# michaelosthege/pytensor-federated

Measured on NVIDIA H100. Metric: logp+grad evals/sec for 8-shard federated GLM, higher is better.
Workload: dtype bf16; 1 GPU; model=federated logistic GLM (logp + gradient), chains_per_eval=1, features=256, global_batch=80000000, seq_len=256, l2_policy=inputs (>= 2.5 GB per GPU) are larger than the 50 MB L2; no flush needed, parallelism=shard-parallel x1 (8 shards/GPU), kernel=auto, backend=fused, comm=local, hbm_bytes_per_eval_per_gpu=31200395264

## Files before the change

pytensor_federated_b200/csrc/glm_tc.cu:

```cuda
#include <cstring>
#include <vector>

#include <cuda.h>
#include <cuda_bf16.h>
#include <cuda_runtime.h>

#include "fed_comm.cuh"
#include "models.h"
#include "tc_common.cuh"
#include "chunks.h"

namespace tc {

constexpr int kTileM = 128;
constexpr int kPanel = 64;
constexpr int kPanelBytes = kTileM * 128;
constexpr int kThreads = 512;
constexpr int kRegs = 65536 / kThreads;
constexpr int kConsumerRegs = 168;
constexpr int kOtherRegs = 88;
static_assert(256 * kConsumerRegs + 256 * kOtherRegs == 65536, "the register split must fill the register file");
constexpr int kConsumerWarps = 8;
constexpr int kMaxChunk = 32;
constexpr int kMinChunk = 4;
constexpr int kRing = 16;
constexpr int kLLRows = 16;

constexpr int kXBlock = kTileM * kPanel * 3 / 2;
constexpr int kXFoot = 256;
constexpr int kXMaxExceptions = kXFoot / 4 - 1;
constexpr int kXSlots = 6;
constexpr int kDecThreads = 224;

__host__ __device__ __forceinline__ uint32_t x12_prmt(uint32_t a, uint32_t b, uint32_t s) {
#ifdef __CUDA_ARCH__
    uint32_t r;
    asm("prmt.b32 %0, %1, %2, %3;" : "=r"(r) : "r"(a), "r"(b), "r"(s));
    return r;
#else
    const uint64_t v = (uint64_t)b << 32 | a;
    uint32_t r = 0;
    for (int k = 0; k < 4; ++k) {
        const uint32_t sel = (s >> (4 * k)) & 0xFu;
        uint32_t byte = (uint32_t)(v >> (8 * (sel & 7u))) & 0xFFu;
        if (sel & 8u) byte = (byte & 0x80u) ? 0xFFu : 0u;
        r |= byte << (8 * k);
    }
    return r;
#endif
}
__host__ __device__ __forceinline__ uint4 x12_decode8(uint2 lo, uint32_t c, const uint32_t (&t)[4]) {
    const uint32_t w = c << 4;
    const uint32_t s0 = c & 0x7777u, s1 = (c >> 16) & 0x7777u;
    const uint32_t m0 = x12_prmt(w, c, 0xD9C8u), m1 = x12_prmt(w, c, 0xFBEAu);
    const uint32_t h0 = (x12_prmt(t[0], t[1], s0) & ~m0) | (x12_prmt(t[2], t[3], s0) & m0);
    const uint32_t h1 = (x12_prmt(t[0], t[1], s1) & ~m1) | (x12_prmt(t[2], t[3], s1) & m1);
    uint4 r;
    r.x = x12_prmt(lo.x, h0, 0x5140u);
    r.y = x12_prmt(lo.x, h0, 0x7362u);
    r.z = x12_prmt(lo.y, h1, 0x5140u);
    r.w = x12_prmt(lo.y, h1, 0x7362u);
    return r;
}
__host__ __device__ __forceinline__ uint32_t x12_chunk_offset(int i) { return (i >> 3) * 128 + (((i & 7) ^ ((i >> 3) & 7)) << 4); }
__host__ __device__ __forceinline__ uint32_t x12_high_byte_offset(uint32_t pos) {
    const uint32_t pnl = pos >> 13, row = (pos >> 6) & 127, f = pos & 63;
    return pnl * kPanelBytes + row * 128 + ((((f >> 3) ^ (row & 7)) << 4) | ((f & 7) << 1)) + 1;
}

struct SmemLayout {
    uint32_t stages, stage_bytes, off_theta_b, theta_b_bytes, off_r, r_bytes, off_rows, row_bytes, off_theta_f,
        off_disp, off_ring, off_bars, total, preload, xslots, xslot_bytes, off_x, off_xfoot;
};
__host__ __device__ inline SmemLayout smem_layout(int P, int n1, int n2, int n_theta, int chain_words, int chains,
                                                  int row_arrays, bool packed = false) {
    SmemLayout L;
    const uint32_t panels = P / kPanel;
    L.stage_bytes = panels * kPanelBytes;
    L.theta_b_bytes = panels * n1 * 128;
    L.r_bytes = kTileM * n2 * 2;
    L.row_bytes = (uint32_t)row_arrays * kTileM * 4;
    const uint32_t bars_bytes = packed ? 256 : 192;
    const uint32_t fixed = L.theta_b_bytes + 2 * L.r_bytes + ((chains * (1 + chain_words) * 4 + 15) & ~15) + kRing * 24 +
                           bars_bytes + (packed ? 2 * kXFoot : 0) + 1024 ;
    uint32_t stages = (227u * 1024u - fixed) / (L.stage_bytes + L.row_bytes);
    if (stages > 4) stages = 4;
    L.xslots = 0;
    L.xslot_bytes = kXBlock + kXFoot + L.row_bytes;
    if (packed) {
        const uint32_t two = fixed + 2 * (L.stage_bytes + L.row_bytes);
        stages = 2;
        if (two <= 227u * 1024u && (uint32_t)n_theta * 4u <= 2u * L.stage_bytes) {
            const uint32_t fit = (227u * 1024u - two) / L.xslot_bytes;
            L.xslots = fit < (uint32_t)kXSlots ? fit : (uint32_t)kXSlots;
        }
    }
    L.stages = stages;
// ... 126 lines not shown
    uint64_t* bar_xempty = bars + 20 + kXSlots;

    const int warp = threadIdx.x >> 5;
    const int lane = threadIdx.x & 31;

    if (threadIdx.x == 0) {
        *pipeline_fault() = 0;
        for (int i = 0; i < kRing; ++i) mbar_init(&bar_ring[i], 1);
        for (int i = 0; i < 4; ++i) { mbar_init(&bar_full[i], PK ? kDecThreads : 1); mbar_init(&bar_empty[i], 32 * kConsumerWarps); }
        if (PK)
            for (int i = 0; i < kXSlots; ++i) { mbar_init(&bar_xfull[i], 1); mbar_init(&bar_xempty[i], kDecThreads); }
        fence_barrier_init();
    }
    if (warp == 0 && lane == 0)
        for (int i = 0; i < prm.n_segments; ++i) {
            tma_prefetch_desc(&tmaps[4 * i]);
            tma_prefetch_desc(&tmaps[4 * i + 1]);
            if (ROWS && segs_g[i].offset) tma_prefetch_desc(&tmaps[4 * i + 2]);
            if (ROWS && segs_g[i].weight) tma_prefetch_desc(&tmaps[4 * i + 3]);
        }
    auto load_tile = [&](int st, int seg, int row0, int rows) {
        const CUtensorMap* m = tmaps + 4 * seg;
        float* slot = reinterpret_cast<float*>(smem + L.off_rows + (size_t)st * L.row_bytes);
        mbar_expect_tx(&bar_full[st], L.stage_bytes + kTileM * 4 * (1 + (rows & 1) + (rows >> 1)));
        for (int pnl = 0; pnl < panels; ++pnl)
            tma_load_2d(smem + (size_t)st * L.stage_bytes + pnl * kPanelBytes, m, pnl * kPanel, row0, &bar_full[st]);
        tma_load_1d(slot, m + 1, row0, &bar_full[st]);
        if (rows & 1) tma_load_1d(slot + o_slot * kTileM, m + 2, row0, &bar_full[st]);
        if (rows & 2) tma_load_1d(slot + w_slot * kTileM, m + 3, row0, &bar_full[st]);
    };
    auto load_xpanel = [&](int xs, int seg, int tile, int pnl, int rows) {
        unsigned char* dst = smem + L.off_x + (size_t)xs * L.xslot_bytes;
        const GlmSegment& g = segs_g[seg];
        const uint32_t extra = pnl == 0 ? kXFoot + kTileM * 4 * (1 + (rows & 1) + (rows >> 1)) : 0;
        mbar_expect_tx(&bar_xfull[xs], kXBlock + extra);
        bulk_load(dst, static_cast<const unsigned char*>(g.xpack) + ((size_t)tile * panels + pnl) * kXBlock, kXBlock, &bar_xfull[xs]);
        if (pnl == 0) {
            const CUtensorMap* m = tmaps + 4 * seg;
            float* slot = reinterpret_cast<float*>(dst + kXBlock + kXFoot);
            bulk_load(dst + kXBlock, static_cast<const unsigned char*>(g.xfoot) + (size_t)tile * kXFoot, kXFoot, &bar_xfull[xs]);
            tma_load_1d(slot, m + 1, tile * kTileM, &bar_xfull[xs]);
            if (rows & 1) tma_load_1d(slot + o_slot * kTileM, m + 2, tile * kTileM, &bar_xfull[xs]);
            if (rows & 2) tma_load_1d(slot + w_slot * kTileM, m + 3, tile * kTileM, &bar_xfull[xs]);
        }
    };
    auto seg_row_mask = [&](int seg) -> int {
        if constexpr (!ROWS) return 0;
        return (segs_g[seg].offset ? 1 : 0) | (segs_g[seg].weight ? 2 : 0);
    };
    unsigned int claim0 = 0;
    int preloaded = 0;
    if (warp == 0) {
        __syncwarp();
        fed::pdl_wait();
        if (lane == 0) claim0 = atomicAdd(work_counter, 1u);
        claim0 = __shfl_sync(0xffffffffu, claim0, 0);
        if (claim0 < (unsigned int)n_chunks) {
            const GlmChunk ch = chunks[claim0];
            const int units = PK ? ch.n_tiles * panels : ch.n_tiles;
            preloaded = units < (int)L.preload ? units : (int)L.preload;
            if (!prm.early_loads) preloaded = 0;
            const int rows = seg_row_mask(ch.seg);
            if (elect_one())
                for (int t = 0; t < preloaded; ++t) {
                    if (PK) load_xpanel(t, ch.seg, ch.first_tile + t / panels, t % panels, rows);
                    else load_tile(t, ch.seg, (ch.first_tile + t) * kTileM, rows);
                }
            __syncwarp();
        }
    }

    __shared__ fed::Prologue s_pro;
    bool active;
    {
// ... 83 lines not shown
                    }
                    __syncwarp();
                    if (!have) break;
                    const int rows = seg_row_mask(ch.seg);
                    for (int t = 0; t < ch.n_tiles && PK; ++t)
                        for (int pnl = 0; pnl < panels; ++pnl) {
                            const int k = t * panels + pnl;
                            if (!(j == 0 && k < preloaded)) {
                                mbar_wait(&bar_xempty[xs.idx], xs.phase ^ 1);
                                if (j == 0 && k == preloaded && lane == 0) fed::stamp(comm, 3);
                                if (elect_one()) load_xpanel(xs.idx, ch.seg, ch.first_tile + t, pnl, rows);
                                __syncwarp();
                            }
                            xs.advance((int)L.xslots);
                        }
                    for (int t = 0; t < ch.n_tiles && !PK; ++t) {
                        const int st = stage.idx;
                        if (j == 0 && t < preloaded) {
                            stage.advance(S);
                            continue;
                        }
                        mbar_wait(&bar_empty[st], stage.phase ^ 1);
                        if (j == 0 && t == preloaded && lane == 0) fed::stamp(comm, 3);
                        if (elect_one()) load_tile(st, ch.seg, (ch.first_tile + t) * kTileM, rows);
                        __syncwarp();
                        stage.advance(S);
                    }
                    claim = __shfl_sync(0xffffffffu, ahead, 0);
                }
                if (lane == 0) fed::stamp(comm, 4);
            } else {
                if (PK) {
                    const int td = warp < 4 ? threadIdx.x - 32 : threadIdx.x - (12 * 32 - 96);
                    constexpr int kDecGroup = KC <= 4 && traits(E).group_panels ? 2 : 1;
                    static_assert(kDecGroup <= 2, "a packed launch may have only 2 compressed slots");
                    int4* decided = reinterpret_cast<int4*>(smem + L.off_bars + 144);
                    Ring stage, xs;
                    uint32_t fb = 0;
                    for (int j = 0;; ++j) {
                        mbar_wait(&bar_ring[j & (kRing - 1)], (uint32_t)((j / kRing) & 1));
                        named_sync(2, kDecThreads);
                        if (td == 0) *decided = *pipeline_fault() ? make_int4(-1, 0, 0, 0) : ring[j & (kRing - 1)];
                        named_sync(2, kDecThreads);
                        const int4 ch = *decided;
                        if (ch.x < 0) break;
                        const uint32_t tab[4] = {segs_g[ch.x].xtab[0], segs_g[ch.x].xtab[1], segs_g[ch.x].xtab[2],
                                                 segs_g[ch.x].xtab[3]};
                        for (int t = 0; t < ch.z; ++t) {
                            mbar_wait(&bar_empty[stage.idx], stage.phase ^ 1);
                            unsigned char* dst = smem + (size_t)stage.idx * L.stage_bytes;
                            int* foot = reinterpret_cast<int*>(smem + L.off_xfoot + fb * kXFoot);
                            for (int pnl = 0; pnl < panels; pnl += kDecGroup) {
                                constexpr int kPer = (kTileM * 8 + kDecThreads - 1) / kDecThreads;
                                uint2 lo[kDecGroup][kPer];
                                uint32_t cw[kDecGroup][kPer];
                                int xi[kDecGroup];
#pragma unroll
                                for (int h = 0; h < kDecGroup; ++h) {
                                    mbar_wait(&bar_xfull[xs.idx], xs.phase);
                                    const unsigned char* src = smem + L.off_x + (size_t)xs.idx * L.xslot_bytes;
                                    if (pnl + h == 0) {
                                        if (td < kXFoot / 4) foot[td] = reinterpret_cast<const int*>(src + kXBlock)[td];
                                        const float* rsrc = reinterpret_cast<const float*>(src + kXBlock + kXFoot);
                                        float* rdst = reinterpret_cast<float*>(smem + L.off_rows + (size_t)stage.idx * L.row_bytes);
                                        for (int i = td; i < (int)L.row_bytes / 4; i += kDecThreads) rdst[i] = rsrc[i];
                                    }
#pragma unroll
                                    for (int k = 0; k < kPer; ++k) {
                                        const int i = td + k * kDecThreads;
                                        if (k < kPer - 1 || i < kTileM * 8) {
                                            lo[h][k] = reinterpret_cast<const uint2*>(src)[i];
                                            cw[h][k] = reinterpret_cast<const uint32_t*>(src + kTileM * kPanel)[i];
                                        }
                                    }
                                    xi[h] = xs.idx;
                                    xs.advance((int)L.xslots);
                                }
#pragma unroll
                                for (int h = 0; h < kDecGroup; ++h) {
                                    unsigned char* pd = dst + (pnl + h) * kPanelBytes;
#pragma unroll
                                    for (int k = 0; k < kPer; ++k) {
                                        const int i = td + k * kDecThreads;
                                        if (k < kPer - 1 || i < kTileM * 8)
                                            *reinterpret_cast<uint4*>(pd + x12_chunk_offset(i)) = x12_decode8(lo[h][k], cw[h][k], tab);
                                    }
                                    mbar_arrive(&bar_xempty[xi[h]]);
                                }
                            }
                            named_sync(2, kDecThreads);
                            const int n_ex = min(foot[0], kXMaxExceptions);
                            for (int e = td; e < n_ex; e += kDecThreads) {
                                const uint32_t v = (uint32_t)foot[1 + e];
                                if ((v >> 8) < (uint32_t)panels * kTileM * kPanel) dst[x12_high_byte_offset(v >> 8)] = (unsigned char)(v & 0xFFu);
                            }
                            fence_proxy_async();
                            mbar_arrive(&bar_full[stage.idx]);
                            stage.advance(S);
                            fb ^= 1u;
                        }
                    }
                }
            }
            named_sync(3, kThreads);
            setmaxnreg<kOtherRegs, kRegs>();
        } else {
            setmaxnreg<kRegs, kConsumerRegs>();
            const int c = (warp >> 2) - 1;
            const int w = warp & 3;
            const int q = lane & 3;
            const int ew = warp - 4;
            const int NB = PP / 128;
            constexpr int NJ = C8 / 8;
            const uint64_t desc_k = make_desc(0, 16, 1024, 1);
            const uint64_t desc_xt = make_desc(0, kPanelBytes, 1024, 1);
            const uint64_t desc_r = make_desc(0, 128, 2048, 0);
            const uint32_t theta_b_a = smem_u32(theta_b);
            const uint32_t x_base_a = smem_u32(smem);
            const uint32_t r_a = smem_u32(r_buf);
// ... 453 lines not shown
    return e == cudaSuccess ? 0 : (int)e;
}

extern "C" int b200_glm_tc_chunk_table(const long long* n_rows, int n_segments, int sm_count, int multiple, int max_chunk,
                                       int min_chunk, int* out, int max_chunks) {
    std::vector<GlmSegment> segs(n_segments);
    for (int s = 0; s < n_segments; ++s) segs[s].n_rows = n_rows[s];
    const std::vector<GlmChunk> chunks = build_chunks(segs.data(), n_segments, sm_count, tc::kTileM, multiple, max_chunk, min_chunk);
    for (size_t i = 0; i < chunks.size() && (int)i < max_chunks; ++i) {
        out[3 * i + 0] = chunks[i].seg;
        out[3 * i + 1] = chunks[i].first_tile;
        out[3 * i + 2] = chunks[i].n_tiles;
    }
    return (int)chunks.size();
}

extern "C" size_t b200_glm_tc_partial_row_doubles(int n_vals, int n_chains, int n_out, int n_groups, int family) {
    return tc::partial_row_doubles(n_vals, chains_bucket(n_chains), n_out > 0 ? n_out : 1, n_groups,
                                   tc::traits(tc::epilogue(family)).disp ? 1 : 0);
}

extern "C" int b200_glm_tc_stages(int n_features, int n_chains, int n_groups, int family, int row_data) {
    const int kc = chains_bucket(n_chains);
    if (kc == 0) return 0;
    return (int)launch_layout(n_features, kc, tc::epilogue(family), 0, row_data != 0, row_data).stages;
}

extern "C" int b200_glm_tc_packed_slots(int n_features, int n_chains, int n_groups, int family, int row_data, int n_theta) {
    const int kc = chains_bucket(n_chains);
    if (kc == 0) return 0;
    return (int)launch_layout(n_features, kc, tc::epilogue(family), n_theta, row_data != 0, row_data, true).xslots;
}

extern "C" int b200_glm_x12_decode_tile(const unsigned char* blocks, const int* footer, const unsigned int* tab, int panels,
                                        unsigned char* out) {
    const uint32_t t[4] = {tab[0], tab[1], tab[2], tab[3]};
    for (int pnl = 0; pnl < panels; ++pnl) {
        const unsigned char* src = blocks + (size_t)pnl * tc::kXBlock;
        for (int i = 0; i < tc::kTileM * 8; ++i) {
            uint2 lo;
            uint32_t c;
            std::memcpy(&lo, src + 8 * i, 8);
            std::memcpy(&c, src + tc::kTileM * tc::kPanel + 4 * i, 4);
            const uint4 v = tc::x12_decode8(lo, c, t);
            std::memcpy(out + (size_t)pnl * tc::kPanelBytes + tc::x12_chunk_offset(i), &v, 16);
        }
    }
    if (footer[0] < 0 || footer[0] > tc::kXMaxExceptions) return -1;
    for (int e = 0; e < footer[0]; ++e) {
        const uint32_t v = (uint32_t)footer[1 + e];
        if ((v >> 8) >= (uint32_t)panels * tc::kTileM * tc::kPanel) return -1;
        out[tc::x12_high_byte_offset(v >> 8)] = (unsigned char)(v & 0xFFu);
    }
    return footer[0];
}

extern "C" int b200_launch_glm_tc(const FedComm* comm, const GlmSegment* segs_dev, const GlmParams* prm, const void* tmaps,
                                  const void* chunks_dev, int n_chunks, unsigned int* work_counter, int grid,
                                  cudaStream_t stream) {
    const int kc = chains_bucket(prm->n_chains);
    if (kc == 0) return -1;
    const bool rows = prm->row_data != 0;
    const LaunchFn fn = pick(tc::epilogue(prm->family), kc, rows);
    if (!fn) return -3;
    return fn(comm, segs_dev, prm, tmaps, chunks_dev, n_chunks, work_counter, grid, stream);
}
```

pytensor_federated_b200/csrc/models.h:

```cpp
#pragma once
#include <cstdint>

struct LinregShard {
    const void* x;
    const void* y;
    long long n;
    double sigma;
    int theta_offset;
    int _pad;
};

struct GlmSegment {
    const void* X;
    const float* y;
    const void* scales;
    const float* offset;
    const float* weight;
    long long n_rows;
    long long first_tile;
    int group;
    int out_group;
    const void* xpack;
    const void* xfoot;
    unsigned int xtab[4];
};

struct GlmParams {
    int n_segments;
    int n_features;
    int ld;
    int n_groups;
    int n_chains;
    int family;
    long long total_tiles;
    int n_out;
    int early_loads;
    int row_data;
    int n_classes;
    int packed_x;
};

constexpr int kGlmRowOffsets = 1;
constexpr int kGlmRowWeights = 2;
constexpr int kGlmHvp = 16;

enum GlmFamilyCode : int {
    kGlmLogistic = 0,
    kGlmPoisson = 1,
    kGlmGaussian = 2,
    kGlmMultinomial = 3,
    kGlmGaussianScale = 4,
    kGlmNegBinomial = 5,
    kGlmOrdinal = 6,
    kGlmWeibull = 7,
    kGlmLogNormal = 8,
    kGlmZeroInflatedPoisson = 9,
    kGlmZeroInflatedNegBinomial = 10,
// ... 57 lines not shown
```

pytensor_federated_b200/csrc/runtime.cu:

```cuda
#include <atomic>
#include <chrono>
#include <cstdio>
#include <cstdlib>
#include <cstring>
#include <string>
#include <thread>
#include <vector>

#include <cuda_runtime.h>

#include "fed_comm.cuh"
#include "models.h"

static bool early_loads_enabled() {
    const char* v = getenv("B200FED_NO_EARLY_LOADS");
    return !(v && *v && *v != '0');
}

extern "C" {
int b200_launch_linreg(const FedComm*, const LinregShard*, int, int, int, cudaStream_t);
int b200_launch_glm_simt(const FedComm*, const GlmSegment*, const GlmParams*, int, cudaStream_t);
size_t b200_glm_simt_smem(int, int, int);
int b200_launch_glm_tc(const FedComm*, const GlmSegment*, const GlmParams*, const void* tmaps, const void* chunks,
                       int n_chunks, unsigned int* work_counter, int grid, cudaStream_t);
// ... 574 lines not shown
    CK(cudaMalloc((void**)&e->glm_segs_dev, sizeof(GlmSegment) * (n_segments > 0 ? n_segments : 1)));
    CK(cudaMemcpy(e->glm_segs_dev, e->glm_segs.data(), sizeof(GlmSegment) * n_segments, cudaMemcpyHostToDevice));
    if (use_tensor_cores == 3 || use_tensor_cores == 4) {
        e->glm_elem_bytes = use_tensor_cores == 3 ? 2 : 4;
        e->kind = MODEL_GLM_GENERIC;
        e->grid = e->sm_count * 2;
    } else if (use_tensor_cores) {
        const bool fp8 = use_tensor_cores == 2;
        if (fp8) {
            int rc = b200_glm_fp8_prepare(e->glm_segs.data(), n_segments, &e->glm, e->sm_count, &e->glm_tmaps_dev,
                                          &e->glm_chunks_dev, &e->glm_n_chunks);
            if (rc != 0) {
                g_last_error = "fp8 GLM path rejected this shape (rc=" + std::to_string(rc) + ")";
                return rc;
            }
        }
        e->tc_row_doubles = fp8 ? b200_glm_fp8_partial_row_doubles(e->n_vals, n_chains, e->glm.n_out, n_groups)
                                : b200_glm_tc_partial_row_doubles(e->n_vals, n_chains, e->glm.n_out, n_groups, family);
        if (e->tc_partials) cudaFree(e->tc_partials);
        const size_t doubles = (size_t)e->sm_count * e->tc_row_doubles + ((size_t)e->sm_count / 16 + 2) * e->n_vals * 2;
        CK(cudaMalloc((void**)&e->tc_partials, doubles * 8));
        CK(cudaMemset(e->tc_partials, 0, doubles * 8));
        e->kind = fp8 ? MODEL_GLM_FP8 : MODEL_GLM_TC;
        e->grid = e->sm_count;
        if (e->glm_n_chunks > 0 && e->grid > e->glm_n_chunks) e->grid = e->glm_n_chunks;
    } else {
        e->kind = MODEL_GLM_SIMT;
        e->grid = e->sm_count * 2;
    }
    if ((long long)e->grid > tiles && tiles > 0) e->grid = (int)tiles;
    return 0;
}

int b200_engine_set_glm_packed(void* h, int n_segments, const void** xpack, const void** xfoot, const unsigned int* tabs) {
    Engine* e = static_cast<Engine*>(h);
    CK(cudaSetDevice(e->device));
    if (e->kind != MODEL_GLM_TC || n_segments != (int)e->glm_segs.size()) {
        g_last_error = "packed X needs the bf16 tensor-core GLM model it was made for";
        return -41;
    }
    std::vector<GlmSegment> segs = e->glm_segs;
    for (int s = 0; s < n_segments; ++s) {
        segs[s].xpack = xpack ? xpack[s] : nullptr;
        segs[s].xfoot = xpack ? xfoot[s] : nullptr;
        for (int q = 0; q < 4; ++q) segs[s].xtab[q] = xpack ? tabs[4 * s + q] : 0u;
        if (xpack && (!segs[s].xpack || !segs[s].xfoot || (((uintptr_t)segs[s].xpack | (uintptr_t)segs[s].xfoot) & 15) != 0)) {
            g_last_error = "packed X: every segment needs 16-byte aligned blocks and footers";
            return -42;
        }
    }
    if (xpack && b200_glm_tc_packed_slots(e->glm.n_features, e->glm.n_chains, e->glm.n_groups, e->glm.family,
                                          e->glm.row_data, e->n_theta) < 2) {
        g_last_error = "packed X: this shape's packed layout does not fit in shared memory";
        return -43;
    }
    CK(cudaMemcpy(e->glm_segs_dev, segs.data(), sizeof(GlmSegment) * n_segments, cudaMemcpyHostToDevice));
    e->glm_segs = segs;
    e->glm.packed_x = xpack ? 1 : 0;
    return 0;
}

void b200_engine_set_custom_launcher(void* h, void* fn) {
    static_cast<Engine*>(h)->custom_launcher =
        reinterpret_cast<int (*)(const FedComm*, const GlmSegment*, const GlmParams*, int, int, cudaStream_t)>(fn);
}

void b200_engine_set_ode_launcher(void* h, void* fn) {
    static_cast<Engine*>(h)->ode_launcher =
        reinterpret_cast<int (*)(const FedComm*, const OdeShard*, int, int, cudaStream_t)>(fn);
}

int b200_engine_set_ode(void* h, int n_shards, const float** t, const float** y0, const float** y_obs, const int* n_series,
                        const int* n_t, const float* sigma, const int* substeps, const int* theta_offset,
                        const int* out_offset) {
    Engine* e = static_cast<Engine*>(h);
    CK(cudaSetDevice(e->device));
    e->ode.resize(n_shards);
    long long series = 0;
    for (int s = 0; s < n_shards; ++s) {
        e->ode[s] = OdeShard{t[s], y0[s], y_obs[s], n_series[s], n_t[s], sigma[s], substeps[s],
// ... 233 lines not shown
```

pytensor_federated_b200/models/glm.py:

```python
from __future__ import annotations

import ctypes as C
import os
from typing import List, Optional, Sequence

import numpy as np

from .base import ShardModel

FAMILIES = {"logistic": 0, "poisson": 1, "gaussian": 2, "multinomial": 3, "gaussian_scale": 4, "negative_binomial": 5,
            "ordinal": 6, "weibull": 7, "lognormal": 8, "zero_inflated_poisson": 9, "zero_inflated_negative_binomial": 10,
            "gamma": 11, "inverse_gaussian": 12, "gaussian_location_scale": 13, "student_t": 14, "beta": 15}


CTA_SMEM_LIMIT = 227 * 1024 - 256


def _family_code(family) -> int:
    return family.code_id if hasattr(family, "code_id") else FAMILIES[family]


def _aligned16(t):
    return t.clone() if t.data_ptr() % 16 != 0 else t

# ... 227 lines not shown
        self.selected_kernel = {0: "simt", 1: "tc", 2: "fp8", 3: "generic-bf16", 4: "generic-fp32"}[code]
        if self.kernel == "auto" and code not in (1, 2) and not hasattr(self.family, "code_id"):
            import logging

            logging.getLogger(__name__).warning(
                "GLM with %d features (%s, row stride %d) is outside the tensor-core kernel's shapes (bf16, P %% 8 == 0, "
                "P <= 384, 16-byte aligned rows): using the %s CUDA-core kernel — single pass, but slower",
                self.n_features, self.Xs[0].dtype, self.ld, self.selected_kernel)
        out_grp = (C.c_int * n)(*self.node_ids) if self.node_ids is not None else None
        op = native.void_p_array([o.data_ptr() if o is not None else 0 for o in self.offsets]) \
            if any(o is not None for o in self.offsets) else None
        wp = native.void_p_array([w.data_ptr() if w is not None else 0 for w in self.weights]) \
            if any(w is not None for w in self.weights) else None
        native.check(
            lib.b200_engine_set_glm(
                handle, n, Xp, yp, sp, rows, grp, self.n_features, self.ld, self.n_groups,
                self.kernel_chains, _family_code(self.family) | (HVP_FLAG if self.hvp else 0), code, out_grp, self.n_nodes, op, wp,
                self.n_classes,
            ),
            "set_glm",
        )
        if hasattr(self.family, "code_id"):
            lib.b200_engine_set_custom_launcher(handle, C.c_void_p(self.family.launcher_address()))
        self.packed_x = False
        if code == 1 and os.environ.get("B200FED_NO_PACKED_X", "0") in ("", "0"):
            row_data = (1 if any(o is not None for o in self.offsets) else 0) | (2 if any(w is not None for w in self.weights) else 0)
            fam = _family_code(self.family) | (HVP_FLAG if self.hvp else 0)
            slots = int(lib.b200_glm_tc_packed_slots(self.n_features, self.kernel_chains, self.n_groups, fam, row_data,
                                                     self.n_theta_words))
            if slots >= 2 and self._packing_pays(row_data):
                packs = self._packed()
                if packs is not None:
                    tabs = (C.c_uint * (4 * n))(*[w for _, _, t in packs for w in t])
                    native.check(lib.b200_engine_set_glm_packed(
                        handle, n, native.void_p_array([p.data_ptr() for p, _, _ in packs]),
                        native.void_p_array([f.data_ptr() for _, f, _ in packs]), tabs), "set_glm_packed")
                    self.packed_x = True

    _packs = None
    _packs_refused = False

    def _packing_pays(self, row_data: int) -> bool:
        return (self.n_features + 127) // 128 == 2 and self.kernel_chains <= X12_MAX_COLUMNS

    def _packed(self):
        import logging

        import torch

        if self._packs is not None or self._packs_refused:
            return self._packs
        log = logging.getLogger(__name__)
        need = sum(x12_packed_bytes(X.shape[0], self.n_features) for X in self.Xs)
        free, _ = torch.cuda.mem_get_info(self.device)
        if need + (2 << 30) > free:
            log.warning("not packing X: it needs %.1f GB and %.1f GB are free; the kernel reads the bf16 matrix",
                        need / 1e9, free / 1e9)
            return None
        packs = []
        for si, X in enumerate(self.Xs):
            p = pack_x12(X[:, : self.n_features])
            if p is None:
                log.warning("not packing X: a tile of segment %d has more than %d values outside its table", si,
                            X12_MAX_EXCEPTIONS)
                self._packs_refused = True
                return None
            packs.append(p)
        self._packs = packs
        return packs

    def reference_partial(self, inputs, *, dtype=None, chunk_rows: int = 1 << 20) -> np.ndarray:
        import torch

        self._last_ctx = self.call_context(inputs)
        return self._partial(inputs, dtype=dtype or torch.float32, chunk_rows=chunk_rows)

    def eager_partial(self, inputs) -> np.ndarray:
        import torch

        if self.Xs[0].dtype != torch.bfloat16:
            return self.reference_partial(inputs)
        self._last_ctx = self.call_context(inputs)
        return self._layout.baseline(self, inputs)

    def _partial(self, inputs, *, dtype, chunk_rows: int, bf16_gemms: bool = False) -> np.ndarray:
        import torch

        lay = self._layout
        icpt, beta, terms = lay.oracle(inputs, self.device, dtype)
        icpt = icpt.to(self.device, dtype)
        B = beta.to(self.device, torch.bfloat16 if bf16_gemms else dtype)
        G, P = self.n_groups, self.n_features
        step = self.kernel_chains // B.shape[1]
        full = torch.zeros(self.n_nodes, self.kernel_chains, 1 + lay.words, dtype=torch.float64, device=self.device)
        for si, (X, y, g) in enumerate(zip(self.Xs, lay.kernel_ys, self.groups)):
            out = full[self.node_ids[si] if self.node_ids is not None else 0]
            w = self.weights[si]
            for r0 in range(0, X.shape[0], chunk_rows):
                r1 = min(X.shape[0], r0 + chunk_rows)
                if bf16_gemms:
                    Xf = X[r0:r1]
                    eta = (Xf @ B).to(dtype)
# ... 9 lines not shown
                out[:, 1 + g] += r.double().sum(0).reshape(-1)
                if not bf16_gemms:
                    out[:, 1 + G : 1 + G + P] += (r.reshape(r1 - r0, -1).T @ Xf).double()
                elif step == 1:
                    out[:, 1 + G : 1 + G + P] += (r.reshape(r1 - r0, -1).T.to(torch.bfloat16) @ Xf).double()
                else:
                    out[::step, 1 + G : 1 + G + P] += (r.sum(2).T.to(torch.bfloat16) @ Xf).double()
                for t in q:
                    out[:, 1 + G + P] += t.double().sum(0).reshape(-1)
        return full.reshape(-1).cpu().numpy()

    def _weigh(self, seg: int, r0: int, r1: int, *terms):
        import torch

        w = self.weights[seg]
        if w is None:
            return terms
        ww = w[r0:r1].to(terms[0].dtype).reshape((-1,) + (1,) * (terms[0].dim() - 1))
        keep = ww != 0
        return [torch.where(keep, ww * t, torch.zeros_like(t)) for t in terms]

    def _dequant_rows(self, seg: int, r0: int, r1: int):
        return self.Xs[seg][r0:r1]

    def _dequant(self, X):
        return X

    def _row_data_bytes(self) -> int:
        return int(sum(4 * v.shape[0] for v in self.offsets + self.weights if v is not None))

    def bytes_per_eval(self) -> int:
        if getattr(self, "packed_x", False):
            xb = sum(x12_packed_bytes(X.shape[0], self.n_features) for X in self.Xs)
            return int(xb + sum(4 * X.shape[0] for X in self.Xs)) + self._row_data_bytes()
        return int(sum(X.shape[0] * (self.n_features * X.element_size() + 4) for X in self.Xs)) + self._row_data_bytes()

    def flops_per_eval(self) -> int:
        return int(4 * self.n_rows * self.n_features * self.kernel_chains)


X12_BLOCK = 128 * 64 * 3 // 2
X12_FOOT = 256
X12_MAX_EXCEPTIONS = X12_FOOT // 4 - 1
X12_MAX_COLUMNS = 4


def x12_tiles(n_rows: int) -> int:
    t = (n_rows + 127) // 128
    return t + (t & 1)


def x12_packed_bytes(n_rows: int, n_features: int) -> int:
    return x12_tiles(n_rows) * (((n_features + 127) // 128 * 2) * X12_BLOCK + X12_FOOT)


def pack_x12(X, chunk_rows: int = 1 << 17):
    import torch

    n, P = X.shape
    PP = (P + 127) // 128 * 128
    panels = PP // 64
    tiles = x12_tiles(n)
    dev = X.device
    hist = torch.zeros(256, dtype=torch.long, device=dev)
    for r0 in range(0, n, chunk_rows):
        hb = (X[r0 : r0 + chunk_rows].contiguous().view(torch.int16) >> 8) & 0xFF
        hist += torch.bincount(hb.reshape(-1).long(), minlength=256)
# ... 6 lines not shown
    for code in range(15 - 1, -1, -1):
        lut[entries[code]] = code
    table = [int.from_bytes(bytes(entries[4 * q : 4 * q + 4]), "little") for q in range(4)]

    blocks = torch.empty(tiles, panels, X12_BLOCK, dtype=torch.uint8, device=dev)
    foot = torch.zeros(tiles, X12_FOOT // 4, dtype=torch.int32, device=dev)
    for r0 in range(0, tiles * 128, chunk_rows):
        rows = min(chunk_rows, tiles * 128 - r0)
        nt = rows // 128
        t0 = r0 // 128
        v = torch.zeros(rows, PP, dtype=torch.int16, device=dev)
        valid = max(0, min(n, r0 + rows) - r0)
        if valid:
            v[:valid, :P] = X[r0 : r0 + valid].view(torch.int16)
        v = v.view(nt, 128, panels, 64).permute(0, 2, 1, 3)
        hb = ((v >> 8) & 0xFF).to(torch.uint8)
        code = lut[hb.long()]
        blocks[t0 : t0 + nt, :, : 8192] = (v & 0xFF).to(torch.uint8).reshape(nt, panels, 8192)
        blocks[t0 : t0 + nt, :, 8192 :] = (code[..., 0::2] | (code[..., 1::2] << 4)).reshape(nt, panels, 4096)
        ex = (code == 15).reshape(nt, panels * 8192)
        cnt = ex.sum(1)
        if int(cnt.max()) > X12_MAX_EXCEPTIONS:
            return None
        foot[t0 : t0 + nt, 0] = cnt.to(torch.int32)
        tile, pos = ex.nonzero(as_tuple=True)
        if tile.numel():
            start = torch.cumsum(cnt, 0) - cnt
            rank = torch.arange(tile.numel(), device=dev) - start[tile]
            word = (pos << 8) | hb.reshape(nt, panels * 8192)[tile, pos].long()
            foot[t0 + tile, 1 + rank] = word.to(torch.int32)
    return blocks, foot, table


def _f64(x):
    import torch

    return torch.as_tensor(np.asarray(x, dtype=np.float64))


def _tc_kernel_only(m) -> None:
    if m.kernel not in ("auto", "tc"):
        raise ValueError(f"kernel={m.kernel!r}: the {m.family} family runs on the bf16 tensor-core kernel only "
                         "(kernel='tc' or 'auto')")


def _check_classes(m, n_classes, most: int, per_chain: int, columns_text: str) -> int:
    if n_classes is None or not 2 <= int(n_classes) <= most:
        raise ValueError(f"the {m.family} family needs n_classes in [2, {most}], got {n_classes}")
    cols = per_chain(int(n_classes))
    if m.n_chains * cols > 16:
        raise ValueError(f"n_chains x {columns_text} must be <= 16 (the tensor-core kernel's columns per launch), got "
                         f"{m.n_chains} x {cols}")
    return int(n_classes)


def _check_integers(m, what: str, valid: str, below) -> None:
    import torch

    for si, (y, w) in enumerate(zip(m.ys, m.weights)):
        bad = ~((y == torch.floor(y)) & (y >= 0) & below(y))
        if w is not None:
            bad &= w != 0
        if bool(torch.any(bad)):
            raise ValueError(f"{what} of segment {si} must be integers in {valid} on every row of non-zero weight")


# ... 1056 lines not shown
```

pytensor_federated_b200/ops/native.py:

```python
from __future__ import annotations

import ctypes as C
import os
from pathlib import Path
from typing import Optional

_PKG = Path(__file__).resolve().parent.parent
LIB_PATH = _PKG / "libb200fed.so"

_lib: Optional[C.CDLL] = None

c_void_pp = C.POINTER(C.c_void_p)
c_ll_p = C.POINTER(C.c_longlong)
c_int_p = C.POINTER(C.c_int)
c_double_p = C.POINTER(C.c_double)
c_float_p = C.POINTER(C.c_float)


class NativeError(RuntimeError):
    pass


def _declare(lib: C.CDLL) -> None:
    def sig(name, restype, *argtypes):
# ... 24 lines not shown
    sig("b200_engine_launches", C.c_ulonglong, C.c_void_p)
    sig("b200_engine_epoch", C.c_ulonglong, C.c_void_p)
    sig("b200_engine_stream", C.c_void_p, C.c_void_p)
    sig("b200_engine_host_theta", C.c_void_p, C.c_void_p)
    sig("b200_engine_host_result", C.c_void_p, C.c_void_p)
    sig(
        "b200_engine_set_linreg", C.c_int, C.c_void_p, C.c_int, c_void_pp, c_void_pp, c_ll_p,
        c_double_p, c_int_p, C.c_int,
    )
    sig(
        "b200_engine_set_glm", C.c_int, C.c_void_p, C.c_int, c_void_pp, c_void_pp, c_void_pp, c_ll_p,
        c_int_p, C.c_int, C.c_int, C.c_int, C.c_int, C.c_int, C.c_int, c_int_p, C.c_int, c_void_pp, c_void_pp,
        C.c_int,
    )
    sig(
        "b200_engine_set_ode", C.c_int, C.c_void_p, C.c_int, c_void_pp, c_void_pp, c_void_pp, c_int_p,
        c_int_p, c_float_p, c_int_p, c_int_p, c_int_p,
    )
    sig("b200_engine_set_custom_launcher", None, C.c_void_p, C.c_void_p)
    sig("b200_engine_set_ode_launcher", None, C.c_void_p, C.c_void_p)
    sig("b200_engine_launch", C.c_int, C.c_void_p)
    sig("b200_engine_set_device_theta", C.c_int, C.c_void_p, C.c_void_p, C.c_int, C.c_int)
    sig("b200_engine_wait", C.c_int, C.c_void_p, C.c_ulonglong, C.c_void_p, C.c_double)
    sig("b200_engine_eval", C.c_int, C.c_void_p, C.c_void_p, C.c_int, C.c_void_p, C.c_double)
    sig("b200_engine_serve", C.c_longlong, C.c_void_p, C.c_int, C.c_longlong)
    sig("b200_engine_stop_serving", None, C.c_void_p)
    sig("b200_engine_stop_peers", C.c_int, C.c_void_p)
    sig("b200_engine_sync", C.c_int, C.c_void_p)
    sig("b200_engine_trace", C.c_int, C.c_void_p, C.c_ulonglong, C.POINTER(C.c_ulonglong))
    sig("b200_glm_tc_chunk_table", C.c_int, c_ll_p, C.c_int, C.c_int, C.c_int, C.c_int, C.c_int, c_int_p, C.c_int)
    sig("b200_glm_tc_stages", C.c_int, C.c_int, C.c_int, C.c_int, C.c_int, C.c_int)
    sig("b200_glm_tc_packed_slots", C.c_int, C.c_int, C.c_int, C.c_int, C.c_int, C.c_int, C.c_int)
    sig("b200_glm_x12_decode_tile", C.c_int, C.c_void_p, C.c_void_p, C.c_void_p, C.c_int, C.c_void_p)
    sig("b200_engine_set_glm_packed", C.c_int, C.c_void_p, C.c_int, c_void_pp, c_void_pp, C.POINTER(C.c_uint))
    sig("b200_engine_enable_cta_trace", None, C.c_void_p, C.c_int)
    sig("b200_engine_cta_trace", C.c_int, C.c_void_p, C.POINTER(C.c_ulonglong), C.c_int)
    sig("b200_engine_destroy", None, C.c_void_p)


def load(build_if_missing: bool = True) -> C.CDLL:
    global _lib
    if _lib is not None:
        return _lib
    if not LIB_PATH.exists() and build_if_missing:
        from .. import build as _build

        _build.build()
    if not LIB_PATH.exists():
        raise NativeError(f"{LIB_PATH} is missing; run `python -m pytensor_federated_b200.build`")
    try:
        lib = C.CDLL(str(LIB_PATH), mode=os.RTLD_NOW | os.RTLD_LOCAL)
    except OSError:
        try:
            import torch

            lib = C.CDLL(str(LIB_PATH), mode=os.RTLD_NOW | os.RTLD_LOCAL)
        except (OSError, ImportError) as ex:
            raise NativeError(f"could not load {LIB_PATH}: {ex}") from ex
    _declare(lib)
    _lib = lib
    return lib


def last_error() -> str:
    return load().b200_last_error().decode("utf-8", "replace")


# ... 18 lines not shown
```

Baseline: 96.74 evals/s.

## Pack binary labels into bitmaps and widen packed-X decoder loads

When the GLM labels are exactly 0/1 floats, the host builds a per-tile 128-bit label bitmap. The packed-X loader then fetches 16 bytes per tile instead of a 512-byte float row, and the decoder threads expand the bits back to floats in shared memory. The decoder is also reorganised so each thread reads paired 16-byte and 8-byte chunks, with its swizzled store offsets hoisted and checked by a compile-time assertion. This cuts HBM label traffic and decoder load instructions, at the cost of a one-time host-side bitmap build and a new API argument.

```diff
diff --git a/pytensor_federated_b200/csrc/glm_tc.cu b/pytensor_federated_b200/csrc/glm_tc.cu
--- a/pytensor_federated_b200/csrc/glm_tc.cu
+++ b/pytensor_federated_b200/csrc/glm_tc.cu
@@ -51,7 +51,7 @@
 }
 __host__ __device__ __forceinline__ uint4 x12_decode8(uint2 lo, uint32_t c, const uint32_t (&t)[4]) {
     const uint32_t w = c << 4;
-    const uint32_t s0 = c & 0x7777u, s1 = (c >> 16) & 0x7777u;
+    const uint32_t s0 = c & 0x77777777u, s1 = s0 >> 16;
     const uint32_t m0 = x12_prmt(w, c, 0xD9C8u), m1 = x12_prmt(w, c, 0xFBEAu);
     const uint32_t h0 = (x12_prmt(t[0], t[1], s0) & ~m0) | (x12_prmt(t[2], t[3], s0) & m0);
     const uint32_t h1 = (x12_prmt(t[0], t[1], s1) & ~m1) | (x12_prmt(t[2], t[3], s1) & m1);
@@ -62,7 +62,24 @@
     r.w = x12_prmt(lo.y, h1, 0x7362u);
     return r;
 }
-__host__ __device__ __forceinline__ uint32_t x12_chunk_offset(int i) { return (i >> 3) * 128 + (((i & 7) ^ ((i >> 3) & 7)) << 4); }
+__host__ __device__ constexpr uint32_t x12_chunk_offset(int i) { return (i >> 3) * 128 + (((i & 7) ^ ((i >> 3) & 7)) << 4); }
+constexpr int kXPerThread = 5;
+constexpr int kXPairChunks = 4 * kDecThreads;
+__host__ __device__ constexpr int x12_thread_chunk(int td, int s) {
+    return s < 4 ? 2 * (td + kDecThreads * (s >> 1)) + (s & 1) : (td < kTileM * 8 - kXPairChunks ? kXPairChunks + td : -1);
+}
+constexpr uint32_t kXPairStride = kDecThreads * 2 / 8 * 128;
+constexpr uint32_t kXTailOffset = kXPairChunks / 8 * 128;
+static_assert([] {
+    for (int td = 0; td < kDecThreads; ++td)
+        for (int s = 0; s < kXPerThread; ++s) {
+            const int i = x12_thread_chunk(td, s);
+            const uint32_t want = s < 4 ? ((s & 1) ? x12_chunk_offset(2 * td) ^ 16u : x12_chunk_offset(2 * td)) + kXPairStride * (s >> 1)
+                                        : x12_chunk_offset(td) + kXTailOffset;
+            if (i >= 0 && x12_chunk_offset(i) != want) return false;
+        }
+    return true;
+}(), "the decoders' hoisted store offsets must be the swizzled chunk offsets");
 __host__ __device__ __forceinline__ uint32_t x12_high_byte_offset(uint32_t pos) {
     const uint32_t pnl = pos >> 13, row = (pos >> 6) & 127, f = pos & 63;
     return pnl * kPanelBytes + row * 128 + ((((f >> 3) ^ (row & 7)) << 4) | ((f & 7) << 1)) + 1;
@@ -255,14 +272,16 @@
     auto load_xpanel = [&](int xs, int seg, int tile, int pnl, int rows) {
         unsigned char* dst = smem + L.off_x + (size_t)xs * L.xslot_bytes;
         const GlmSegment& g = segs_g[seg];
-        const uint32_t extra = pnl == 0 ? kXFoot + kTileM * 4 * (1 + (rows & 1) + (rows >> 1)) : 0;
+        const unsigned int* ybits = pnl == 0 ? g.ybits : nullptr;
+        const uint32_t extra = pnl == 0 ? kXFoot + (ybits ? 16 : kTileM * 4) + kTileM * 4 * ((rows & 1) + (rows >> 1)) : 0;
         mbar_expect_tx(&bar_xfull[xs], kXBlock + extra);
         bulk_load(dst, static_cast<const unsigned char*>(g.xpack) + ((size_t)tile * panels + pnl) * kXBlock, kXBlock, &bar_xfull[xs]);
         if (pnl == 0) {
             const CUtensorMap* m = tmaps + 4 * seg;
             float* slot = reinterpret_cast<float*>(dst + kXBlock + kXFoot);
             bulk_load(dst + kXBlock, static_cast<const unsigned char*>(g.xfoot) + (size_t)tile * kXFoot, kXFoot, &bar_xfull[xs]);
-            tma_load_1d(slot, m + 1, tile * kTileM, &bar_xfull[xs]);
+            if (ybits) bulk_load(slot, ybits + (size_t)tile * 4, 16, &bar_xfull[xs]);
+            else tma_load_1d(slot, m + 1, tile * kTileM, &bar_xfull[xs]);
             if (rows & 1) tma_load_1d(slot + o_slot * kTileM, m + 2, tile * kTileM, &bar_xfull[xs]);
             if (rows & 2) tma_load_1d(slot + w_slot * kTileM, m + 3, tile * kTileM, &bar_xfull[xs]);
         }
@@ -412,6 +431,7 @@
             } else {
                 if (PK) {
                     const int td = warp < 4 ? threadIdx.x - 32 : threadIdx.x - (12 * 32 - 96);
+                    const uint32_t so0 = x12_chunk_offset(2 * td), so1 = so0 ^ 16u, sot = x12_chunk_offset(td);
                     constexpr int kDecGroup = KC <= 4 && traits(E).group_panels ? 2 : 1;
                     static_assert(kDecGroup <= 2, "a packed launch may have only 2 compressed slots");
                     int4* decided = reinterpret_cast<int4*>(smem + L.off_bars + 144);
@@ -426,14 +446,16 @@
                         if (ch.x < 0) break;
                         const uint32_t tab[4] = {segs_g[ch.x].xtab[0], segs_g[ch.x].xtab[1], segs_g[ch.x].xtab[2],
                                                  segs_g[ch.x].xtab[3]};
+                        const bool ybits = segs_g[ch.x].ybits != nullptr;
                         for (int t = 0; t < ch.z; ++t) {
                             mbar_wait(&bar_empty[stage.idx], stage.phase ^ 1);
                             unsigned char* dst = smem + (size_t)stage.idx * L.stage_bytes;
                             int* foot = reinterpret_cast<int*>(smem + L.off_xfoot + fb * kXFoot);
                             for (int pnl = 0; pnl < panels; pnl += kDecGroup) {
-                                constexpr int kPer = (kTileM * 8 + kDecThreads - 1) / kDecThreads;
-                                uint2 lo[kDecGroup][kPer];
-                                uint32_t cw[kDecGroup][kPer];
+                                uint4 lo[kDecGroup][2];
+                                uint2 cw[kDecGroup][2];
+                                uint2 lt[kDecGroup];
+                                uint32_t ct[kDecGroup];
                                 int xi[kDecGroup];
 #pragma unroll
                                 for (int h = 0; h < kDecGroup; ++h) {
@@ -443,15 +465,18 @@
                                         if (td < kXFoot / 4) foot[td] = reinterpret_cast<const int*>(src + kXBlock)[td];
                                         const float* rsrc = reinterpret_cast<const float*>(src + kXBlock + kXFoot);
                                         float* rdst = reinterpret_cast<float*>(smem + L.off_rows + (size_t)stage.idx * L.row_bytes);
-                                        for (int i = td; i < (int)L.row_bytes / 4; i += kDecThreads) rdst[i] = rsrc[i];
+                                        const uint32_t* bits = reinterpret_cast<const uint32_t*>(rsrc);
+                                        for (int i = td; i < (int)L.row_bytes / 4; i += kDecThreads)
+                                            rdst[i] = ybits && i < kTileM ? (float)((bits[i >> 5] >> (i & 31)) & 1u) : rsrc[i];
                                     }
 #pragma unroll
-                                    for (int k = 0; k < kPer; ++k) {
-                                        const int i = td + k * kDecThreads;
-                                        if (k < kPer - 1 || i < kTileM * 8) {
-                                            lo[h][k] = reinterpret_cast<const uint2*>(src)[i];
-                                            cw[h][k] = reinterpret_cast<const uint32_t*>(src + kTileM * kPanel)[i];
-                                        }
+                                    for (int k = 0; k < 2; ++k) {
+                                        lo[h][k] = reinterpret_cast<const uint4*>(src)[td + k * kDecThreads];
+                                        cw[h][k] = reinterpret_cast<const uint2*>(src + kTileM * kPanel)[td + k * kDecThreads];
+                                    }
+                                    if (td < kTileM * 8 - kXPairChunks) {
+                                        lt[h] = reinterpret_cast<const uint2*>(src)[kXPairChunks + td];
+                                        ct[h] = reinterpret_cast<const uint32_t*>(src + kTileM * kPanel)[kXPairChunks + td];
                                     }
                                     xi[h] = xs.idx;
                                     xs.advance((int)L.xslots);
@@ -460,11 +485,14 @@
                                 for (int h = 0; h < kDecGroup; ++h) {
                                     unsigned char* pd = dst + (pnl + h) * kPanelBytes;
 #pragma unroll
-                                    for (int k = 0; k < kPer; ++k) {
-                                        const int i = td + k * kDecThreads;
-                                        if (k < kPer - 1 || i < kTileM * 8)
-                                            *reinterpret_cast<uint4*>(pd + x12_chunk_offset(i)) = x12_decode8(lo[h][k], cw[h][k], tab);
+                                    for (int k = 0; k < 2; ++k) {
+                                        *reinterpret_cast<uint4*>(pd + so0 + kXPairStride * k) =
+                                            x12_decode8(make_uint2(lo[h][k].x, lo[h][k].y), cw[h][k].x, tab);
+                                        *reinterpret_cast<uint4*>(pd + so1 + kXPairStride * k) =
+                                            x12_decode8(make_uint2(lo[h][k].z, lo[h][k].w), cw[h][k].y, tab);
                                     }
+                                    if (td < kTileM * 8 - kXPairChunks)
+                                        *reinterpret_cast<uint4*>(pd + sot + kXTailOffset) = x12_decode8(lt[h], ct[h], tab);
                                     mbar_arrive(&bar_xempty[xi[h]]);
                                 }
                             }
@@ -984,19 +1012,29 @@
     return (int)launch_layout(n_features, kc, tc::epilogue(family), n_theta, row_data != 0, row_data, true).xslots;
 }
 
+extern "C" int b200_glm_x12_thread_chunks(int* out, int n) {
+    for (int td = 0; td < tc::kDecThreads; ++td)
+        for (int s = 0; s < tc::kXPerThread; ++s)
+            if (td * tc::kXPerThread + s < n) out[td * tc::kXPerThread + s] = tc::x12_thread_chunk(td, s);
+    return tc::kDecThreads * tc::kXPerThread;
+}
+
 extern "C" int b200_glm_x12_decode_tile(const unsigned char* blocks, const int* footer, const unsigned int* tab, int panels,
                                         unsigned char* out) {
     const uint32_t t[4] = {tab[0], tab[1], tab[2], tab[3]};
     for (int pnl = 0; pnl < panels; ++pnl) {
         const unsigned char* src = blocks + (size_t)pnl * tc::kXBlock;
-        for (int i = 0; i < tc::kTileM * 8; ++i) {
-            uint2 lo;
-            uint32_t c;
-            std::memcpy(&lo, src + 8 * i, 8);
-            std::memcpy(&c, src + tc::kTileM * tc::kPanel + 4 * i, 4);
-            const uint4 v = tc::x12_decode8(lo, c, t);
-            std::memcpy(out + (size_t)pnl * tc::kPanelBytes + tc::x12_chunk_offset(i), &v, 16);
-        }
+        for (int td = 0; td < tc::kDecThreads; ++td)
+            for (int s = 0; s < tc::kXPerThread; ++s) {
+                const int i = tc::x12_thread_chunk(td, s);
+                if (i < 0) continue;
+                uint2 lo;
+                uint32_t c;
+                std::memcpy(&lo, src + 8 * i, 8);
+                std::memcpy(&c, src + tc::kTileM * tc::kPanel + 4 * i, 4);
+                const uint4 v = tc::x12_decode8(lo, c, t);
+                std::memcpy(out + (size_t)pnl * tc::kPanelBytes + tc::x12_chunk_offset(i), &v, 16);
+            }
     }
     if (footer[0] < 0 || footer[0] > tc::kXMaxExceptions) return -1;
     for (int e = 0; e < footer[0]; ++e) {
diff --git a/pytensor_federated_b200/csrc/models.h b/pytensor_federated_b200/csrc/models.h
--- a/pytensor_federated_b200/csrc/models.h
+++ b/pytensor_federated_b200/csrc/models.h
@@ -23,6 +23,7 @@
     const void* xpack;
     const void* xfoot;
     unsigned int xtab[4];
+    const unsigned int* ybits;
 };
 
 struct GlmParams {
diff --git a/pytensor_federated_b200/csrc/runtime.cu b/pytensor_federated_b200/csrc/runtime.cu
--- a/pytensor_federated_b200/csrc/runtime.cu
+++ b/pytensor_federated_b200/csrc/runtime.cu
@@ -630,7 +630,8 @@
     return 0;
 }
 
-int b200_engine_set_glm_packed(void* h, int n_segments, const void** xpack, const void** xfoot, const unsigned int* tabs) {
+int b200_engine_set_glm_packed(void* h, int n_segments, const void** xpack, const void** xfoot, const unsigned int* tabs,
+                               const void** ybits) {
     Engine* e = static_cast<Engine*>(h);
     CK(cudaSetDevice(e->device));
     if (e->kind != MODEL_GLM_TC || n_segments != (int)e->glm_segs.size()) {
@@ -642,8 +643,10 @@
         segs[s].xpack = xpack ? xpack[s] : nullptr;
         segs[s].xfoot = xpack ? xfoot[s] : nullptr;
         for (int q = 0; q < 4; ++q) segs[s].xtab[q] = xpack ? tabs[4 * s + q] : 0u;
-        if (xpack && (!segs[s].xpack || !segs[s].xfoot || (((uintptr_t)segs[s].xpack | (uintptr_t)segs[s].xfoot) & 15) != 0)) {
-            g_last_error = "packed X: every segment needs 16-byte aligned blocks and footers";
+        segs[s].ybits = xpack && ybits ? static_cast<const unsigned int*>(ybits[s]) : nullptr;
+        if (xpack && (!segs[s].xpack || !segs[s].xfoot ||
+                      (((uintptr_t)segs[s].xpack | (uintptr_t)segs[s].xfoot | (uintptr_t)segs[s].ybits) & 15) != 0)) {
+            g_last_error = "packed X: every segment needs 16-byte aligned blocks, footers and label bitmaps";
             return -42;
         }
     }
diff --git a/pytensor_federated_b200/models/glm.py b/pytensor_federated_b200/models/glm.py
--- a/pytensor_federated_b200/models/glm.py
+++ b/pytensor_federated_b200/models/glm.py
@@ -283,13 +283,15 @@
                 packs = self._packed()
                 if packs is not None:
                     tabs = (C.c_uint * (4 * n))(*[w for _, _, t in packs for w in t])
+                    bits = native.void_p_array([b.data_ptr() if b is not None else 0 for b in self._label_bits()])
                     native.check(lib.b200_engine_set_glm_packed(
                         handle, n, native.void_p_array([p.data_ptr() for p, _, _ in packs]),
-                        native.void_p_array([f.data_ptr() for _, f, _ in packs]), tabs), "set_glm_packed")
+                        native.void_p_array([f.data_ptr() for _, f, _ in packs]), tabs, bits), "set_glm_packed")
                     self.packed_x = True
 
     _packs = None
     _packs_refused = False
+    _ybits = None
 
     def _packing_pays(self, row_data: int) -> bool:
         return (self.n_features + 127) // 128 == 2 and self.kernel_chains <= X12_MAX_COLUMNS
@@ -319,6 +321,16 @@
             packs.append(p)
         self._packs = packs
         return packs
+
+    def _label_bits(self):
+        if self._ybits is None:
+            made = {}
+            for y in self._layout.kernel_ys:
+                key = (y.data_ptr(), y.shape[0])
+                if key not in made:
+                    made[key] = x12_label_bits(y)
+            self._ybits = [made[(y.data_ptr(), y.shape[0])] for y in self._layout.kernel_ys]
+        return self._ybits
 
     def reference_partial(self, inputs, *, dtype=None, chunk_rows: int = 1 << 20) -> np.ndarray:
         import torch
@@ -394,7 +406,8 @@
     def bytes_per_eval(self) -> int:
         if getattr(self, "packed_x", False):
             xb = sum(x12_packed_bytes(X.shape[0], self.n_features) for X in self.Xs)
-            return int(xb + sum(4 * X.shape[0] for X in self.Xs)) + self._row_data_bytes()
+            yb = sum(4 * X.shape[0] if b is None else b.numel() * 4 for X, b in zip(self.Xs, self._label_bits()))
+            return int(xb + yb) + self._row_data_bytes()
         return int(sum(X.shape[0] * (self.n_features * X.element_size() + 4) for X in self.Xs)) + self._row_data_bytes()
 
     def flops_per_eval(self) -> int:
@@ -467,6 +480,22 @@
     return blocks, foot, table
 
 
+def x12_label_bits(y):
+    import torch
+
+    if y.dtype != torch.float32:
+        return None
+    v = y.contiguous().view(torch.int32)
+    one = v == 0x3F800000
+    if not bool((one | (v == 0)).all()):
+        return None
+    tiles = x12_tiles(y.shape[0])
+    flags = torch.zeros(tiles * 128, dtype=torch.int64, device=y.device)
+    flags[: y.shape[0]] = one.to(torch.int64)
+    words = (flags.view(tiles * 4, 32) << torch.arange(32, device=y.device)).sum(1)
+    return torch.where(words >= 1 << 31, words - (1 << 32), words).to(torch.int32).view(tiles, 4)
+
+
 def _f64(x):
     import torch
 
diff --git a/pytensor_federated_b200/ops/native.py b/pytensor_federated_b200/ops/native.py
--- a/pytensor_federated_b200/ops/native.py
+++ b/pytensor_federated_b200/ops/native.py
@@ -80,7 +80,8 @@
     sig("b200_glm_tc_stages", C.c_int, C.c_int, C.c_int, C.c_int, C.c_int, C.c_int)
     sig("b200_glm_tc_packed_slots", C.c_int, C.c_int, C.c_int, C.c_int, C.c_int, C.c_int, C.c_int)
     sig("b200_glm_x12_decode_tile", C.c_int, C.c_void_p, C.c_void_p, C.c_void_p, C.c_int, C.c_void_p)
-    sig("b200_engine_set_glm_packed", C.c_int, C.c_void_p, C.c_int, c_void_pp, c_void_pp, C.POINTER(C.c_uint))
+    sig("b200_glm_x12_thread_chunks", C.c_int, c_int_p, C.c_int)
+    sig("b200_engine_set_glm_packed", C.c_int, C.c_void_p, C.c_int, c_void_pp, c_void_pp, C.POINTER(C.c_uint), c_void_pp)
     sig("b200_engine_enable_cta_trace", None, C.c_void_p, C.c_int)
     sig("b200_engine_cta_trace", C.c_int, C.c_void_p, C.POINTER(C.c_ulonglong), C.c_int)
     sig("b200_engine_destroy", None, C.c_void_p)
```

Result: faster. 99.06 evals/s (median of 6 runs) (+2.4%).
